# nju-websoft/OpenEA

Hardware: AMD Instinct MI355X
Metric: training triples/sec (k=10 truncated negatives + limited loss + Adagrad) (higher is better)
Workload: dtype f32; 1 GPU; BootEA/AlignE translational step, EN-FR-100K-V1 shape (synthetic), dim=100, GLOBAL batch=20000 positives (weak scaling: 20000 per GPU x 1 GPU), k=10, truncated eps=0.98; the same workload at every N (; global_batch=20000, entities=200000, parallelism=single

## Files before the change

### openea_amd/csrc/sampler.hip

```cpp
#include <stdlib.h>

#include <algorithm>

#include "common.h"

namespace {

__global__ void tripleset_clear(uint64_t *table, uint64_t capacity) {
    for (uint64_t i = (uint64_t)blockIdx.x * blockDim.x + threadIdx.x; i < capacity; i += (uint64_t)gridDim.x * blockDim.x)
        table[i] = OEA_EMPTY_KEY;
}

__global__ void tripleset_insert(const int32_t *__restrict__ triples, int64_t n, uint64_t *table, uint64_t capacity) {
    for (int64_t i = (int64_t)blockIdx.x * blockDim.x + threadIdx.x; i < n; i += (int64_t)gridDim.x * blockDim.x) {
        const uint64_t key = oea::pack_triple((uint32_t)triples[3 * i], (uint32_t)triples[3 * i + 1], (uint32_t)triples[3 * i + 2]);
        uint64_t s = oea::mix64(key) & (capacity - 1);
        for (;;) {
            const unsigned long long prev = atomicCAS((unsigned long long *)&table[s], (unsigned long long)OEA_EMPTY_KEY, (unsigned long long)key);
            if (prev == OEA_EMPTY_KEY || prev == key) break;
            s = (s + 1) & (capacity - 1);
        }
    }
}

__device__ __forceinline__ uint64_t filter_bit(uint64_t key, uint64_t bits) { return oea::mix64(key ^ 0x9E3779B97F4A7C15ull) & (bits - 1); }

__global__ void tripleset_filter_insert(const int32_t *__restrict__ triples, int64_t n, uint32_t *__restrict__ filter, uint64_t bits) {
    for (int64_t i = (int64_t)blockIdx.x * blockDim.x + threadIdx.x; i < n; i += (int64_t)gridDim.x * blockDim.x) {
        const uint64_t b = filter_bit(oea::pack_triple((uint32_t)triples[3 * i], (uint32_t)triples[3 * i + 1], (uint32_t)triples[3 * i + 2]), bits);
        atomicOr(&filter[b >> 5], 1u << (b & 31));
    }
}

__device__ __forceinline__ bool contains(const uint64_t *__restrict__ table, uint64_t capacity, const uint32_t *__restrict__ filter,
                                         uint64_t filter_bits, uint32_t h, uint32_t r, uint32_t t) {
    const uint64_t key = oea::pack_triple(h, r, t);
    if (filter) {
        const uint64_t b = filter_bit(key, filter_bits);
        if (!((filter[b >> 5] >> (b & 31)) & 1u)) return false;
    }
    uint64_t s = oea::mix64(key) & (capacity - 1);
    for (;;) {
        const uint64_t cur = table[s];
        if (cur == key) return true;
        if (cur == OEA_EMPTY_KEY) return false;
        s = (s + 1) & (capacity - 1);
    }
}

constexpr int kMaxK = 64;

template <int G>
__global__ __launch_bounds__(256) void sample_negatives_kernel(
    const int32_t *__restrict__ pos, int64_t n_pos, int64_t n_split, int k, oea_sampler_side side0,
    oea_sampler_side side1, uint32_t k0, uint32_t k1, uint32_t step, uint32_t pos_offset,
    int max_try, int32_t *__restrict__ out, int32_t *__restrict__ err_flag,
    const int64_t *__restrict__ seg_off, const int64_t *__restrict__ seg_split, int n_seg, const int32_t *__restrict__ replay) {
    const int lane = threadIdx.x % G;
    const uint32_t step_in = step;
    const int64_t n_split_in = n_split;
    for (int64_t p = ((int64_t)blockIdx.x * blockDim.x + threadIdx.x) / G; p < n_pos; p += (int64_t)gridDim.x * blockDim.x / G) {
    step = step_in;
    n_split = n_split_in;
    int64_t pl = p;
    if (seg_off) {
        const int64_t p0 = ((int64_t)(uint32_t)__builtin_amdgcn_readfirstlane((int)(p >> 32)) << 32) | (uint32_t)__builtin_amdgcn_readfirstlane((int)p);
        int lo = 0, hi = n_seg;
        while (hi - lo > 1) {
            const int mid = (lo + hi) >> 1;
            if (seg_off[mid] <= p0) lo = mid; else hi = mid;
        }
        int64_t first = seg_off[lo], split = seg_split[lo];
        int seg = lo;
        if (p >= seg_off[lo + 1]) {
            int l2 = lo;
            hi = n_seg;
            while (hi - l2 > 1) {
                const int mid = (l2 + hi) >> 1;
                if (seg_off[mid] <= p) l2 = mid; else hi = mid;
            }
            seg = l2; first = seg_off[l2]; split = seg_split[l2];
        }
        pl = p - first;
        n_split = split;
        step += (uint32_t)seg;
    }
    const oea_sampler_side &sd = pl < n_split ? side0 : side1;
    const uint64_t *__restrict__ table = sd.table;
    const uint64_t capacity = sd.capacity;
    const int32_t *__restrict__ entity_list = sd.entity_list;
    const int32_t *__restrict__ ent_pos = sd.ent_pos;
    const int32_t *__restrict__ nbr = sd.nbr;
    const uint32_t *__restrict__ filter = sd.filter;
    const uint64_t filter_bits = sd.filter_bits;
    const int n_ent_list = sd.n_ent_list, nbr_k = sd.nbr_k;
    const int32_t h = pos[3 * p], r = pos[3 * p + 1], t = pos[3 * p + 2];
    const bool h_has = nbr && ent_pos[h] >= 0, t_has = nbr && ent_pos[t] >= 0;
    const int32_t *hc = h_has ? nbr + (int64_t)ent_pos[h] * nbr_k : entity_list;
    const int32_t *tc = t_has ? nbr + (int64_t)ent_pos[t] * nbr_k : entity_list;
    const int hn = h_has ? nbr_k : n_ent_list, tn = t_has ? nbr_k : n_ent_list;
    const uint32_t c0 = (uint32_t)pl + pos_offset;
    const int gbase = (threadIdx.x & 63) / G * G;
    const unsigned long long gmask = (G == 64 ? ~0ull : ((1ull << G) - 1ull)) << gbase;
    int got = 0;
    for (int tr = 0; tr < max_try && got < k; ++tr) {
        const bool spare = k < G;
        uint4 w = oea::philox4x32_10(c0, step, (uint32_t)tr, (spare && lane != G - 1) ? 1u + (uint32_t)lane : 0u, k0, k1);
        const uint32_t side_word = spare ? (uint32_t)__shfl((int)w.x, (int)((threadIdx.x & 63) / G * G) + G - 1, 64) : w.x;
        const int32_t *rp = replay ? replay + ((int64_t)p * max_try + tr) * (1 + k) : nullptr;
        const bool corrupt_head = rp ? rp[0] != 0 : (side_word & 1u) != 0u;
        const int32_t *cand = corrupt_head ? hc : tc;
        const int nc = corrupt_head ? hn : tn;
        const int need = k - got;
        if (need > nc) { if (lane == 0) *err_flag = 1; break; }
        const bool active = lane < need;
        uint32_t att = 0;
        int32_t v = -1 - lane;
        if (active) {
            if (!spare) w = oea::philox4x32_10(c0, step, (uint32_t)tr, 1u + (uint32_t)lane, k0, k1);
            v = rp ? rp[1 + lane] : (int32_t)__umulhi(w.x, (uint32_t)nc);
            if (rp && (v < 0 || v >= nc)) { *err_flag = 2; v = 0; }
        }
        for (;;) {
            bool conflict = false;
            for (int q = 0; q < need; ++q) {
                const int32_t vq = __shfl(v, gbase + q, 64);
                conflict |= (q < lane) && (vq == v);
            }
            conflict &= active;
            if ((__ballot(conflict) & gmask) == 0ull) break;
            if (conflict) {
                ++att;
                w = oea::philox4x32_10(c0, step, (uint32_t)tr, 1u + (uint32_t)lane + 64u * att, k0, k1);
                v = (int32_t)__umulhi(w.x, (uint32_t)nc);
            }
        }
        bool accept = false;
        int32_t nh = h, nt = t;
        if (active) {
            const int32_t e = cand[v];
            nh = corrupt_head ? e : h;
            nt = corrupt_head ? t : e;
            accept = (tr == max_try - 1) || !contains(table, capacity, filter, filter_bits, (uint32_t)nh, (uint32_t)r, (uint32_t)nt);
        }
        const unsigned long long acc_mask = (__ballot(accept) & gmask) >> gbase;
        if (accept) {
            const int slot = got + __popcll(acc_mask & ((1ull << lane) - 1ull));
            struct __attribute__((packed, aligned(4))) Triple { int32_t h, r, t; };
            *reinterpret_cast<Triple *>(out + ((int64_t)p * k + slot) * 3) = Triple{nh, r, nt};
        }
        got += __popcll(acc_mask);
    }
    }
}

}

extern "C" {

uint64_t oea_tripleset_capacity(int64_t n) {
    uint64_t cap = 16;
    while (cap < 2ull * (uint64_t)(n > 1 ? n : 1)) cap *= 2;
    return cap;
}

int oea_tripleset_build(const int32_t *triples, int64_t n, uint64_t *table, uint64_t capacity, void *stream) {
    OEA_REQUIRE(table && (triples || n == 0), "null pointer");
    OEA_REQUIRE(capacity >= 2ull * (uint64_t)n && (capacity & (capacity - 1)) == 0, "capacity: power of two >= 2n");
    hipStream_t st = oea::as_stream(stream);
    tripleset_clear<<<1024, 256, 0, st>>>(table, capacity);
    if (n > 0) tripleset_insert<<<(unsigned)std::min<int64_t>(oea::ceil_div(n, 256), 4096), 256, 0, st>>>(triples, n, table, capacity);
    OEA_CHECK_HIP(hipGetLastError());
    return OEA_OK;
}

uint64_t oea_tripleset_filter_bits(uint64_t capacity) { return 8ull * capacity; }

int oea_tripleset_filter_build(const int32_t *triples, int64_t n, uint32_t *filter, uint64_t filter_bits, void *stream) {
    OEA_REQUIRE(filter && (triples || n == 0), "null pointer");
    OEA_REQUIRE(filter_bits >= 32 && (filter_bits & (filter_bits - 1)) == 0, "filter_bits: a power of two >= 32");
    hipStream_t st = oea::as_stream(stream);
    OEA_CHECK_HIP(hipMemsetAsync(filter, 0, (size_t)(filter_bits / 8), st));
    if (n > 0) tripleset_filter_insert<<<(unsigned)std::min<int64_t>(oea::ceil_div(n, 256), 4096), 256, 0, st>>>(triples, n, filter, filter_bits);
    OEA_CHECK_HIP(hipGetLastError());
    return OEA_OK;
}

int oea_sample_negatives(const int32_t *pos, int64_t n_pos, int32_t k, const uint64_t *table,
                         uint64_t capacity, const int32_t *entity_list, int32_t n_ent_list,
                         const int32_t *ent_pos, const int32_t *nbr, int32_t nbr_k, uint64_t seed,
                         uint32_t step, uint32_t pos_offset, int32_t max_try, int32_t *out,
                         int32_t *err_flag, void *stream) {
    oea_sampler_side sd{};
    sd.table = table; sd.capacity = capacity; sd.entity_list = entity_list; sd.ent_pos = ent_pos; sd.nbr = nbr;
    sd.n_ent_list = n_ent_list; sd.nbr_k = nbr_k;
    return oea_sample_negatives_pair(pos, n_pos, n_pos, k, &sd, &sd, seed, step, pos_offset, max_try, out, err_flag,
                                     stream);
}

static int check_side(const oea_sampler_side *s, int k) {
    OEA_REQUIRE(s && s->table && s->entity_list, "sampler side: null pointer");
    OEA_REQUIRE(s->nbr == nullptr || (s->ent_pos != nullptr && s->nbr_k > 0), "nbr needs ent_pos and nbr_k");
    OEA_REQUIRE((s->nbr ? s->nbr_k : s->n_ent_list) >= k && s->n_ent_list >= k, "Sample larger than population");
    return OEA_OK;
}

static int sample_impl(const int32_t *pos, int64_t n_pos, int64_t n_split, int32_t k,
                       const oea_sampler_side *side0, const oea_sampler_side *side1, uint64_t seed,
                       uint32_t step, uint32_t pos_offset, int32_t max_try, int32_t *out,
                       int32_t *err_flag, const int64_t *seg_off_dev, const int64_t *seg_split_dev, int n_seg,
                       void *stream, const int32_t *replay = nullptr) {
    OEA_REQUIRE(pos && out && err_flag, "null pointer");
    OEA_REQUIRE(k >= 1 && k <= kMaxK, "1 <= k <= 64");
    OEA_REQUIRE(max_try >= 1, "max_try >= 1");
    OEA_REQUIRE(n_split >= 0 && n_split <= n_pos, "0 <= n_split <= n_pos");
    int rc = check_side(side0, k);
    if (rc != OEA_OK) return rc;
    rc = check_side(side1, k);
    if (rc != OEA_OK) return rc;
    if (n_pos == 0) return OEA_OK;
    hipStream_t st = oea::as_stream(stream);
    static const int64_t cap_env = [] { const char *e = getenv("OEA_SAMPLER_CAP"); return e ? (int64_t)atoll(e) : (int64_t)0; }();
    const int64_t cap = (seg_off_dev && cap_env > 0) ? cap_env : ((int64_t)1 << 30);
    if (k <= 16)
        sample_negatives_kernel<16><<<(unsigned)std::min<int64_t>(oea::ceil_div(n_pos, 256 / 16), cap), 256, 0, st>>>(
            pos, n_pos, n_split, k, *side0, *side1, (uint32_t)seed, (uint32_t)(seed >> 32), step, pos_offset, max_try,
            out, err_flag, seg_off_dev, seg_split_dev, n_seg, replay);
    else
        sample_negatives_kernel<64><<<(unsigned)std::min<int64_t>(oea::ceil_div(n_pos, 256 / 64), cap), 256, 0, st>>>(
            pos, n_pos, n_split, k, *side0, *side1, (uint32_t)seed, (uint32_t)(seed >> 32), step, pos_offset, max_try,
            out, err_flag, seg_off_dev, seg_split_dev, n_seg, replay);
    OEA_CHECK_HIP(hipGetLastError());
    return OEA_OK;
}

int oea_sample_negatives_pair(const int32_t *pos, int64_t n_pos, int64_t n_split, int32_t k,
                              const oea_sampler_side *side0, const oea_sampler_side *side1, uint64_t seed,
                              uint32_t step, uint32_t pos_offset, int32_t max_try, int32_t *out,
                              int32_t *err_flag, void *stream) {
    return sample_impl(pos, n_pos, n_split, k, side0, side1, seed, step, pos_offset, max_try, out, err_flag, nullptr,
                       nullptr, 0, stream);
}

int oea_sample_negatives_replay(const int32_t *pos, int64_t n_pos, int32_t k, const uint64_t *table, uint64_t capacity,
                                const int32_t *entity_list, int32_t n_ent_list, const int32_t *ent_pos, const int32_t *nbr,
                                int32_t nbr_k, int32_t max_try, const int32_t *replay, int32_t *out, int32_t *err_flag, void *stream) {
    OEA_REQUIRE(replay, "replay record");
    oea_sampler_side sd{};
    sd.table = table; sd.capacity = capacity; sd.entity_list = entity_list; sd.ent_pos = ent_pos; sd.nbr = nbr;
    sd.n_ent_list = n_ent_list; sd.nbr_k = nbr_k;
    return sample_impl(pos, n_pos, n_pos, k, &sd, &sd, 0, 0u, 0u, max_try, out, err_flag, nullptr, nullptr, 0, stream, replay);
}

int oea_sample_negatives_epoch(const int32_t *pos_all, int64_t n_rows, const int64_t *offsets_dev,
                               const int64_t *splits_dev, int32_t steps, int32_t k, const oea_sampler_side *side0,
                               const oea_sampler_side *side1, uint64_t seed, uint32_t step_base, int32_t max_try,
                               int32_t *out_all, int32_t *err_flag, void *stream) {
    OEA_REQUIRE(offsets_dev && splits_dev && steps >= 1, "offsets / splits / steps");
    return sample_impl(pos_all, n_rows, 0, k, side0, side1, seed, step_base, 0u, max_try, out_all, err_flag, offsets_dev,
                       splits_dev, steps, stream);
}

}
```

Baseline: 295.6 million triples/s.

## Add grouped negative sampler kernel processing two positives per lane group

Adds a new sampling kernel where each 16-lane group handles two positive triples at once, batching the first try's loads (positive triple, neighbour row, candidate entity, bloom filter word, hash-table probe) across them. The goal is more memory-level parallelism so dependent gather latencies overlap instead of running back-to-back. Positives that fall short of k after the first try drop back to the original per-try loop. It is the default for k<=16 without replay and can be turned off through an environment variable, at the price of more registers and a more complex code path.

```diff
diff --git a/openea_amd/csrc/sampler.hip b/openea_amd/csrc/sampler.hip
--- a/openea_amd/csrc/sampler.hip
+++ b/openea_amd/csrc/sampler.hip
@@ -49,43 +49,23 @@
 }
 
 constexpr int kMaxK = 64;
+constexpr int kSamplerGroup = 2;
+
+struct __attribute__((packed, aligned(4))) Triple { int32_t h, r, t; };
+
+__device__ __forceinline__ int find_batch(const int64_t *__restrict__ seg_off, int lo, int hi, int64_t p) {
+    while (hi - lo > 1) {
+        const int mid = (lo + hi) >> 1;
+        if (seg_off[mid] <= p) lo = mid; else hi = mid;
+    }
+    return lo;
+}
 
 template <int G>
-__global__ __launch_bounds__(256) void sample_negatives_kernel(
-    const int32_t *__restrict__ pos, int64_t n_pos, int64_t n_split, int k, oea_sampler_side side0,
-    oea_sampler_side side1, uint32_t k0, uint32_t k1, uint32_t step, uint32_t pos_offset,
-    int max_try, int32_t *__restrict__ out, int32_t *__restrict__ err_flag,
-    const int64_t *__restrict__ seg_off, const int64_t *__restrict__ seg_split, int n_seg, const int32_t *__restrict__ replay) {
+__device__ __forceinline__ void sample_rounds(const int32_t *__restrict__ pos, int64_t p, uint32_t c0, uint32_t step, const oea_sampler_side &sd,
+                                              int k, uint32_t k0, uint32_t k1, int max_try, int32_t *__restrict__ out,
+                                              int32_t *__restrict__ err_flag, const int32_t *__restrict__ replay, int tr_begin, int got) {
     const int lane = threadIdx.x % G;
-    const uint32_t step_in = step;
-    const int64_t n_split_in = n_split;
-    for (int64_t p = ((int64_t)blockIdx.x * blockDim.x + threadIdx.x) / G; p < n_pos; p += (int64_t)gridDim.x * blockDim.x / G) {
-    step = step_in;
-    n_split = n_split_in;
-    int64_t pl = p;
-    if (seg_off) {
-        const int64_t p0 = ((int64_t)(uint32_t)__builtin_amdgcn_readfirstlane((int)(p >> 32)) << 32) | (uint32_t)__builtin_amdgcn_readfirstlane((int)p);
-        int lo = 0, hi = n_seg;
-        while (hi - lo > 1) {
-            const int mid = (lo + hi) >> 1;
-            if (seg_off[mid] <= p0) lo = mid; else hi = mid;
-        }
-        int64_t first = seg_off[lo], split = seg_split[lo];
-        int seg = lo;
-        if (p >= seg_off[lo + 1]) {
-            int l2 = lo;
-            hi = n_seg;
-            while (hi - l2 > 1) {
-                const int mid = (l2 + hi) >> 1;
-                if (seg_off[mid] <= p) l2 = mid; else hi = mid;
-            }
-            seg = l2; first = seg_off[l2]; split = seg_split[l2];
-        }
-        pl = p - first;
-        n_split = split;
-        step += (uint32_t)seg;
-    }
-    const oea_sampler_side &sd = pl < n_split ? side0 : side1;
     const uint64_t *__restrict__ table = sd.table;
     const uint64_t capacity = sd.capacity;
     const int32_t *__restrict__ entity_list = sd.entity_list;
@@ -99,14 +79,12 @@
     const int32_t *hc = h_has ? nbr + (int64_t)ent_pos[h] * nbr_k : entity_list;
     const int32_t *tc = t_has ? nbr + (int64_t)ent_pos[t] * nbr_k : entity_list;
     const int hn = h_has ? nbr_k : n_ent_list, tn = t_has ? nbr_k : n_ent_list;
-    const uint32_t c0 = (uint32_t)pl + pos_offset;
     const int gbase = (threadIdx.x & 63) / G * G;
     const unsigned long long gmask = (G == 64 ? ~0ull : ((1ull << G) - 1ull)) << gbase;
-    int got = 0;
-    for (int tr = 0; tr < max_try && got < k; ++tr) {
+    for (int tr = tr_begin; tr < max_try && got < k; ++tr) {
         const bool spare = k < G;
         uint4 w = oea::philox4x32_10(c0, step, (uint32_t)tr, (spare && lane != G - 1) ? 1u + (uint32_t)lane : 0u, k0, k1);
-        const uint32_t side_word = spare ? (uint32_t)__shfl((int)w.x, (int)((threadIdx.x & 63) / G * G) + G - 1, 64) : w.x;
+        const uint32_t side_word = spare ? (uint32_t)__shfl((int)w.x, gbase + G - 1, 64) : w.x;
         const int32_t *rp = replay ? replay + ((int64_t)p * max_try + tr) * (1 + k) : nullptr;
         const bool corrupt_head = rp ? rp[0] != 0 : (side_word & 1u) != 0u;
         const int32_t *cand = corrupt_head ? hc : tc;
@@ -146,12 +124,202 @@
         const unsigned long long acc_mask = (__ballot(accept) & gmask) >> gbase;
         if (accept) {
             const int slot = got + __popcll(acc_mask & ((1ull << lane) - 1ull));
-            struct __attribute__((packed, aligned(4))) Triple { int32_t h, r, t; };
             *reinterpret_cast<Triple *>(out + ((int64_t)p * k + slot) * 3) = Triple{nh, r, nt};
         }
         got += __popcll(acc_mask);
     }
-    }
+}
+
+template <int G>
+__global__ __launch_bounds__(256) void sample_negatives_kernel(
+    const int32_t *__restrict__ pos, int64_t n_pos, int64_t n_split, int k, oea_sampler_side side0,
+    oea_sampler_side side1, uint32_t k0, uint32_t k1, uint32_t step, uint32_t pos_offset,
+    int max_try, int32_t *__restrict__ out, int32_t *__restrict__ err_flag,
+    const int64_t *__restrict__ seg_off, const int64_t *__restrict__ seg_split, int n_seg, const int32_t *__restrict__ replay) {
+    const uint32_t step_in = step;
+    const int64_t n_split_in = n_split;
+    for (int64_t p = ((int64_t)blockIdx.x * blockDim.x + threadIdx.x) / G; p < n_pos; p += (int64_t)gridDim.x * blockDim.x / G) {
+        step = step_in;
+        n_split = n_split_in;
+        int64_t pl = p;
+        if (seg_off) {
+            const int64_t p0 = ((int64_t)(uint32_t)__builtin_amdgcn_readfirstlane((int)(p >> 32)) << 32) | (uint32_t)__builtin_amdgcn_readfirstlane((int)p);
+            const int lo = find_batch(seg_off, 0, n_seg, p0);
+            int64_t first = seg_off[lo], split = seg_split[lo];
+            int seg = lo;
+            if (p >= seg_off[lo + 1]) {
+                seg = find_batch(seg_off, lo, n_seg, p);
+                first = seg_off[seg]; split = seg_split[seg];
+            }
+            pl = p - first;
+            n_split = split;
+            step += (uint32_t)seg;
+        }
+        sample_rounds<G>(pos, p, (uint32_t)pl + pos_offset, step, pl < n_split ? side0 : side1, k, k0, k1, max_try, out, err_flag, replay, 0, 0);
+    }
+}
+
+template <int U, bool NBR>
+__global__ __launch_bounds__(256) void sample_negatives_grouped_kernel(
+    const int32_t *__restrict__ pos, int64_t n_pos, int64_t n_split_in, int k, oea_sampler_side side0,
+    oea_sampler_side side1, uint32_t k0, uint32_t k1, uint32_t step_in, uint32_t pos_offset,
+    int max_try, int32_t *__restrict__ out, int32_t *__restrict__ err_flag,
+    const int64_t *__restrict__ seg_off, const int64_t *__restrict__ seg_split, int n_seg) {
+    constexpr int G = 16, kTile = 256 / G * U;
+    const int lane = threadIdx.x % G, grp = threadIdx.x / G;
+    const int gbase = (threadIdx.x & 63) / G * G;
+    const unsigned long long gmask = ((1ull << G) - 1ull) << gbase;
+    const bool spare = k < G, active = lane < k, last0 = max_try == 1;
+    const bool use_filter = side0.filter && side1.filter;
+    const int64_t n_tiles = (n_pos + kTile - 1) / kTile;
+    for (int64_t tile = blockIdx.x; tile < n_tiles; tile += gridDim.x) {
+        const int64_t p0 = tile * kTile;
+        int lo = 0;
+        int64_t first0 = 0, split0 = n_split_in, next0 = n_pos;
+        if (seg_off) {
+            lo = find_batch(seg_off, 0, n_seg, p0);
+            first0 = seg_off[lo]; split0 = seg_split[lo]; next0 = seg_off[lo + 1];
+        }
+        int64_t p[U];
+        Triple tri[U];
+#pragma unroll
+        for (int u = 0; u < U; ++u) {
+            p[u] = p0 + u * (256 / G) + grp;
+            tri[u] = *reinterpret_cast<const Triple *>(pos + 3 * std::min<int64_t>(p[u], n_pos - 1));
+        }
+        uint32_t c0[U], step[U], draw[U];
+        bool is1[U], head[U];
+#pragma unroll
+        for (int u = 0; u < U; ++u) {
+            const int64_t pq = std::min<int64_t>(p[u], n_pos - 1);
+            int seg = lo;
+            int64_t first = first0, split = split0;
+            if (pq >= next0) {
+                seg = find_batch(seg_off, lo, n_seg, pq);
+                first = seg_off[seg]; split = seg_split[seg];
+            }
+            c0[u] = (uint32_t)(pq - first) + pos_offset;
+            step[u] = step_in + (uint32_t)seg;
+            is1[u] = pq - first >= split;
+            uint4 w = oea::philox4x32_10(c0[u], step[u], 0u, (spare && lane != G - 1) ? 1u + (uint32_t)lane : 0u, k0, k1);
+            const uint32_t side_word = spare ? (uint32_t)__shfl((int)w.x, gbase + G - 1, 64) : w.x;
+            if (!spare) w = oea::philox4x32_10(c0[u], step[u], 0u, 1u + (uint32_t)lane, k0, k1);
+            head[u] = (side_word & 1u) != 0u;
+            draw[u] = w.x;
+        }
+        int32_t row[U];
+#pragma unroll
+        for (int u = 0; u < U; ++u) {
+            row[u] = -1;
+            if (NBR) row[u] = (is1[u] ? side1.ent_pos : side0.ent_pos)[head[u] ? tri[u].h : tri[u].t];
+        }
+        __builtin_amdgcn_sched_barrier(0);
+        const int32_t *cand[U];
+        int32_t v[U];
+        bool bad[U];
+#pragma unroll
+        for (int u = 0; u < U; ++u) {
+            const oea_sampler_side &sd = is1[u] ? side1 : side0;
+            const bool has = row[u] >= 0;
+            cand[u] = has ? sd.nbr + (int64_t)row[u] * sd.nbr_k : sd.entity_list;
+            const int nc = has ? sd.nbr_k : sd.n_ent_list;
+            bad[u] = k > nc;
+            v[u] = (active && !bad[u]) ? (int32_t)__umulhi(draw[u], (uint32_t)nc) : -1 - lane;
+            uint32_t att = 0;
+            for (;;) {
+                bool conflict = false;
+                for (int q = 0; q < k; ++q) {
+                    const int32_t vq = __shfl(v[u], gbase + q, 64);
+                    conflict |= (q < lane) && (vq == v[u]);
+                }
+                conflict &= active;
+                if ((__ballot(conflict) & gmask) == 0ull) break;
+                if (conflict) {
+                    ++att;
+                    const uint4 w = oea::philox4x32_10(c0[u], step[u], 0u, 1u + (uint32_t)lane + 64u * att, k0, k1);
+                    v[u] = (int32_t)__umulhi(w.x, (uint32_t)nc);
+                }
+            }
+            if (bad[u]) v[u] = 0;
+        }
+        bool accept[U];
+        int32_t e[U];
+#pragma unroll
+        for (int u = 0; u < U; ++u) { accept[u] = false; e[u] = 0; }
+        if (active) {
+#pragma unroll
+            for (int u = 0; u < U; ++u) e[u] = cand[u][v[u]];
+            uint64_t key[U];
+            bool maybe[U];
+#pragma unroll
+            for (int u = 0; u < U; ++u) {
+                key[u] = oea::pack_triple((uint32_t)(head[u] ? e[u] : tri[u].h), (uint32_t)tri[u].r, (uint32_t)(head[u] ? tri[u].t : e[u]));
+                maybe[u] = true;
+            }
+            if (use_filter) {
+                uint32_t word[U];
+#pragma unroll
+                for (int u = 0; u < U; ++u) {
+                    const uint64_t b = filter_bit(key[u], is1[u] ? side1.filter_bits : side0.filter_bits);
+                    word[u] = (is1[u] ? side1.filter : side0.filter)[b >> 5] >> (b & 31);
+                }
+#pragma unroll
+                for (int u = 0; u < U; ++u) maybe[u] = (word[u] & 1u) != 0u;
+            }
+            uint64_t cur[U], s[U];
+#pragma unroll
+            for (int u = 0; u < U; ++u) {
+                s[u] = maybe[u] ? oea::mix64(key[u]) & ((is1[u] ? side1.capacity : side0.capacity) - 1) : 0;
+                cur[u] = (is1[u] ? side1.table : side0.table)[s[u]];
+            }
+#pragma unroll
+            for (int u = 0; u < U; ++u) {
+                bool present = false;
+                if (maybe[u]) {
+                    const uint64_t *__restrict__ table = is1[u] ? side1.table : side0.table;
+                    const uint64_t capacity = is1[u] ? side1.capacity : side0.capacity;
+                    for (;;) {
+                        if (cur[u] == key[u]) { present = true; break; }
+                        if (cur[u] == OEA_EMPTY_KEY) break;
+                        s[u] = (s[u] + 1) & (capacity - 1);
+                        cur[u] = table[s[u]];
+                    }
+                }
+                accept[u] = (last0 || !present) && !bad[u] && p[u] < n_pos;
+            }
+        }
+        int got[U];
+        unsigned short_of_k = 0;
+#pragma unroll
+        for (int u = 0; u < U; ++u) {
+            const unsigned long long acc_mask = (__ballot(accept[u]) & gmask) >> gbase;
+            if (accept[u]) {
+                const int slot = __popcll(acc_mask & ((1ull << lane) - 1ull));
+                *reinterpret_cast<Triple *>(out + ((int64_t)p[u] * k + slot) * 3) =
+                    Triple{head[u] ? e[u] : tri[u].h, tri[u].r, head[u] ? tri[u].t : e[u]};
+            }
+            got[u] = __popcll(acc_mask);
+            if (p[u] < n_pos && bad[u] && lane == 0) *err_flag = 1;
+            if (p[u] < n_pos && !bad[u] && got[u] < k) short_of_k |= 1u << u;
+        }
+        while (short_of_k) {
+            const int u_next = __ffs(short_of_k) - 1;
+            short_of_k &= short_of_k - 1;
+            int64_t pp = p[0];
+            uint32_t cc = c0[0], ss = step[0];
+            bool ii = is1[0];
+            int gg = got[0];
+#pragma unroll
+            for (int u = 1; u < U; ++u)
+                if (u == u_next) { pp = p[u]; cc = c0[u]; ss = step[u]; ii = is1[u]; gg = got[u]; }
+            sample_rounds<G>(pos, pp, cc, ss, ii ? side1 : side0, k, k0, k1, max_try, out, err_flag, nullptr, 1, gg);
+        }
+    }
+}
+
+template <int U, bool NBR, class... A>
+void launch_grouped(int64_t n_pos, int64_t cap, hipStream_t st, A... args) {
+    sample_negatives_grouped_kernel<U, NBR><<<(unsigned)std::min<int64_t>(oea::ceil_div(n_pos, 256 / 16 * U), cap), 256, 0, st>>>(args...);
 }
 
 }
@@ -222,7 +390,19 @@
     hipStream_t st = oea::as_stream(stream);
     static const int64_t cap_env = [] { const char *e = getenv("OEA_SAMPLER_CAP"); return e ? (int64_t)atoll(e) : (int64_t)0; }();
     const int64_t cap = (seg_off_dev && cap_env > 0) ? cap_env : ((int64_t)1 << 30);
-    if (k <= 16)
+    const char *group_str = getenv("OEA_SAMPLER_GROUP");
+    const int group_env = (group_str && atoi(group_str) == 1) ? 1 : kSamplerGroup;
+    const bool nbr = side0->nbr != nullptr;
+    const int group = (k > 16 || replay || nbr != (side1->nbr != nullptr)) ? 1 : group_env;
+    if (group != 1) {
+        const uint32_t k0 = (uint32_t)seed, k1 = (uint32_t)(seed >> 32);
+        if (nbr)
+            launch_grouped<kSamplerGroup, true>(n_pos, cap, st, pos, n_pos, n_split, k, *side0, *side1, k0, k1, step, pos_offset, max_try, out,
+                                                err_flag, seg_off_dev, seg_split_dev, n_seg);
+        else
+            launch_grouped<kSamplerGroup, false>(n_pos, cap, st, pos, n_pos, n_split, k, *side0, *side1, k0, k1, step, pos_offset, max_try, out,
+                                                 err_flag, seg_off_dev, seg_split_dev, n_seg);
+    } else if (k <= 16)
         sample_negatives_kernel<16><<<(unsigned)std::min<int64_t>(oea::ceil_div(n_pos, 256 / 16), cap), 256, 0, st>>>(
             pos, n_pos, n_split, k, *side0, *side1, (uint32_t)seed, (uint32_t)(seed >> 32), step, pos_offset, max_try,
             out, err_flag, seg_off_dev, seg_split_dev, n_seg, replay);
```

Measured after the change: 303.3 million triples/s (median of 6 runs). 1.03x the previous value.
